# Fancomi2017/InstanceFusion

Hardware: AMD Instinct MI355X
Metric: frames/s + ms/frame (ICP|fuse|instance) at 640x480, 5M surfels, 1/2/4/8 GPU (higher is better)
Workload: dtype f32; 1 GPU; 5000000-surfel map, 640x480 synthetic RGBD stream, 3-level ICP+RGB + surfel fuse + canned-mask instance votes with superpixel refinement; surfels_live=4734799, surfel_slots=4734799, map_order=random, parallelism=replicas x1, loop_frames=90

## Files before the change

### instancefusion_amd/csrc/ifx_api.hip

```cpp
#include <climits>
#include "ifx_ctx.h"
#include <string.h>
#include <stdio.h>
#include <algorithm>

int ifx_tracker_external_pose(ifx* h, const float* d_pose16, float weight_mult);
int ifx_tracker_set_weight(ifx* h, float weight_mult);
int ifx_compact_enqueue(ifx* h, int refresh_ids);

void hs_invalidate_view(ifx* h);
static std::string g_err;
extern "C" const char* ifx_global_error(void) { return g_err.c_str(); }
extern "C" const char* ifx_last_error(ifx_t* h) { return h ? h->err.c_str() : g_err.c_str(); }

hipEvent_t ifx_event_get(ifx* h)
{
    if (!h->event_pool.empty()) { hipEvent_t e = h->event_pool.back(); h->event_pool.pop_back(); return e; }
    hipEvent_t e;
    hipEventCreate(&e);
    return e;
}
void ifx_ktime_begin(ifx* h, const char* name, hipEvent_t* a)
{
    (void)name;
// ... 285 lines not shown
    else if (s == "stage_timing") h->opt_stage_timing = value;
    else if (s == "track_ahead") h->opt_track_ahead = value;
    else if (s == "slic_ahead") h->opt_slic_ahead = value;
    else if (s == "fold_result") h->opt_fold_result = value;
    else if (s == "clean_raster") h->opt_clean_raster = value;
    else if (s == "hot_records") { h->opt_hot = value; h->hot_valid = 0; }
    else if (s == "hot_verify") h->opt_hot_verify = value;
    else if (s == "own_first_live") h->opt_own_first_live = value;
    else if (s == "own_track_rows") {
        if (!h->own) { h->err = "own_track_rows: the handle was not created for a sharded map"; return IFX_E_STATE; }
        h->opt_own_track_rows = value;
    }
    else if (s == "own_track_rows_emulate") h->opt_own_track_rows_emulate = value;
    else if (s == "own_key_rs") {
        if (!h->own) { h->err = "own_key_rs: the handle was not created for a sharded map"; return IFX_E_STATE; }
        if (h->own_g * 8 > IFX_KEY_SLACK) { h->err = "own_key_rs: more ranks than the key image's slack allows"; return IFX_E_INVALID; }
        h->opt_own_key_rs = value;
    }
    else if (s == "own_lazy_ids") {
        if (!h->own) { h->err = "own_lazy_ids: the handle was not created for a sharded map"; return IFX_E_STATE; }
        if (value && ifx_own_lattice(h) + 1 > 16 * 1024) { h->err = "own_lazy_ids: the image's id lattice is larger than the pack kernel's one workgroup holds (16 383 entries)"; return IFX_E_INVALID; }
        h->opt_own_lazy_ids = value;
    }
    else if (s == "id_rule") {
        if (value != 0 && value != 1) { h->err = "id_rule must be 0 (ray-disc) or 1 (the reference's screen-space quads)"; return IFX_E_INVALID; }
        if (h->own || h->shard_n > 1) { h->err = "id_rule: the id renders of a sharded map keep the ray-disc rule"; return IFX_E_STATE; }
        if (h->hint_rgb || h->slot[h->tick & 1].for_tick == h->tick || h->ids_pending || h->clean_raster_pending) { h->err = "id_rule cannot change while a frame is in flight or announced ahead"; return IFX_E_STATE; }
        if (value != h->opt_id_rule) {
            h->opt_id_rule = value;
            h->ids_full_valid = 0; h->ids_sparse_frame = 1; h->ids_view_ok = 0;
            h->seg_counts_valid = 0;
            const int r = ifx_ids_ensure(h);
            if (r) return r;
        }
    }
    else if (s == "cam_swap") h->opt_cam_swap = value;
    else if (s == "cam_side") h->opt_cam_side = value;
    else if (s == "host_entry_async") h->opt_host_entry_async = value;
    else if (s == "gn_prologue_blocks") h->opt_gn_prologue_blocks = value;
    else if (s == "compact_divisor") h->opt_compact_divisor = value;
    else if (s == "icp_blocks") h->opt_icp_blocks = std::max(0, std::min(2048, value));
    else if (s == "view_blocks") h->opt_view_blocks = std::max(0, std::min(65536, value));
    else if (s == "clean_blocks") h->opt_clean_blocks = std::max(0, std::min(65536, value));
    else if (s == "index_blocks") h->opt_index_blocks = std::max(0, std::min(8192, value));
    else if (s == "res_blocks") h->opt_res_blocks = std::max(0, std::min(4096, value));
    else if (s == "rgb_blocks") h->opt_rgb_blocks = std::max(0, std::min(1024, value));
    else if (s == "raster_tiles") h->opt_raster_tiles = value;
    else if (s == "view_list") { h->opt_vlist = value; ifx_vlist_reap(h); hs_invalidate_view(h); }
    else if (s == "seg_aside") h->opt_seg_aside = value;
    else if (s == "pace") h->opt_pace = value;
    else if (s == "lazy_ids") { ifx_ids_ensure(h); h->opt_lazy_ids = value; }
    else if (s == "seg_device") h->opt_seg_device = value;
    else if (s == "compare_map") {
        if (value != 1 && value != 2) { h->err = "compare_map must be 1 (box IoU) or 2 (mask IoU)"; return IFX_E_INVALID; }
        if (value == 2 && (h->own || h->shard_n > 1)) { h->err = "compare_map 2: the mask rule is not offered on a sharded map (dilated presence is not additive over ranks)"; return IFX_E_STATE; }
        h->opt_compare_map = value;
    }
    else if (s == "seg_snapshots") { if (value < 1 || value > 8) { h->err = "seg_snapshots must be in [1, 8]"; return IFX_E_INVALID; } h->opt_seg_snapshots = value; }
    else if (s == "ff_rounds") h->opt_ff_rounds = value;
    else if (s == "gn_persist_blocks") { if (value < 1) return IFX_E_INVALID; ifx_drop_tracked(h); h->opt_gn_persist_blocks = value; }
    else if (s == "gn_persist") {
        if (value < 0 || value > 7) { h->err = "gn_persist is a mask of pyramid levels (0..7)"; return IFX_E_INVALID; }
        ifx_drop_tracked(h);
        h->opt_gn_persist = value;
    }
    else if (s == "gn_spin_limit" || s == "gn_fault") {
        if (value < 0) return IFX_E_INVALID;
        ifx_drop_tracked(h);
        HIPCHK(h, hipStreamSynchronize(h->stream));
        HIPCHK(h, hipMemcpy((char*)h->d_state + (s == "gn_fault" ? offsetof(DevState, gn_fault) : offsetof(DevState, gn_spin_limit)), &value, sizeof(int), hipMemcpyHostToDevice));
    }
    else if (s == "gn_prologue") { ifx_drop_tracked(h); h->opt_gn_prologue = value ? 1 : 0; }
    else if (s == "rgb_cand") { ifx_drop_tracked(h); h->opt_rgb_cand = value ? 1 : 0; }
    else if (s == "rgb_fuse") {
        if (value < 0 || value > 7) { h->err = "rgb_fuse is a mask of pyramid levels (0..7)"; return IFX_E_INVALID; }
        ifx_drop_tracked(h);
        h->opt_rgb_fuse = value;
    }
    else if (s == "rgb_fuse_poll") { ifx_drop_tracked(h); h->opt_rgb_fuse_poll = value ? 1 : 0; }
    else if (s == "rgb_own") {
        if (value < 0 || value > 7) { h->err = "rgb_own is a mask of pyramid levels (0..7)"; return IFX_E_INVALID; }
        ifx_drop_tracked(h);
        h->opt_rgb_own = value;
    }
    else if (s == "raster_lds") h->opt_raster_lds = value;
    else if (s == "raster_earlyz") h->opt_raster_earlyz = value;
    else if (s == "pyramid" || s == "fast_odom" || s == "so3" || s == "icp_weight_x1000") {
        if (h->hint_rgb || h->slot[h->tick & 1].for_tick == h->tick) { h->err = "tracker options cannot change while a frame is announced ahead"; return IFX_E_STATE; }
        ifx_drop_tracked(h);
        if (s == "pyramid") h->cfg.pyramid = value ? 1 : 0;
        else if (s == "fast_odom") h->cfg.fast_odom = value ? 1 : 0;
        else if (s == "so3") h->cfg.so3 = value ? 1 : 0;
        else { if (value < 0 || value > 100000) { h->err = "icp_weight_x1000 must be in [0, 100000]"; return IFX_E_INVALID; } h->cfg.icp_weight = value / 1000.f; }
    }
    else { h->err = "unknown option " + s; return IFX_E_INVALID; }
    return IFX_OK;
}

__global__ void k_frame_result(DevState* __restrict__ st, FrameResult* __restrict__ out, float* __restrict__ traj_slot)
{
    if (threadIdx.x < 64) frame_result_wave(st, out, traj_slot, 0, (int)threadIdx.x);
}

static int enqueue_frame_side(ifx* h, int s, int tick, const uint8_t* rgb, const uint16_t* depth, int src_kind)
{
    FrameSlot& f = h->slot[s];
    const int bound = h->cur_slot;
    hipStream_t q = h->opt_two_streams ? h->stream_b : h->stream;
    if (q != h->stream) HIPCHK(h, hipStreamWaitEvent(q, f.released, 0));
    if (f.snap_pending) { if (q != h->stream) HIPCHK(h, hipStreamWaitEvent(q, f.snap_read, 0)); f.snap_pending = 0; }
    h->cur = q;
    ifx_bind_slot(h, s);
    hipMemcpyKind kind = src_kind ? hipMemcpyHostToDevice : hipMemcpyDeviceToDevice;
    hipError_t e2 = hipMemcpyAsync(f.depth_raw, depth, (size_t)h->P * 2, kind, q), e1 = hipSuccess;
    if (e2 == hipSuccess) {
        StageTimer t(h, 3);
        ifx_preprocess(h);
        if (h->late_rgb_src && src_kind == 1) { memcpy(h->rgb_stage, h->late_rgb_src, (size_t)h->P * 3); h->late_rgb_src = nullptr; }
        e1 = hipMemcpyAsync(f.rgb, rgb, (size_t)h->P * 3, kind, q);
        if (e1 == hipSuccess) ifx_tracker_frame_side(h, tick == 1);
    }
    hipEventRecord(f.ready, q);
    f.for_tick = tick; f.src_rgb = rgb; f.src_depth = depth;
    h->cur = h->stream;
    ifx_bind_slot(h, bound);
    if (e1 != hipSuccess || e2 != hipSuccess) { h->err = "frame copy failed"; return IFX_E_HIP; }
    return IFX_OK;
}

int ifx_enqueue_hinted_frame_side(ifx* h)
{
    if (!h->hint_rgb || !h->opt_two_streams) { h->hint_rgb = nullptr; return IFX_OK; }
    const uint8_t* r = h->hint_rgb; const uint16_t* d = h->hint_depth;
    const int kind = h->hint_kind;
    h->hint_rgb = nullptr; h->hint_depth = nullptr; h->hint_kind = 0;
    if (h->stream_b && h->slot[h->tick & 1].ready) HIPCHK(h, hipStreamWaitEvent(h->stream_b, h->slot[h->tick & 1].ready, 0));
    int rr = enqueue_frame_side(h, (h->tick + 1) & 1, h->tick + 1, r, d, kind);
    if (!rr && kind == 1) h->prestaged_tick = h->tick + 1;
    return rr;
}

__global__ void k_lc_idle(DevState* st, float* __restrict__ host_lc)
{
    if (threadIdx.x != 0) return;
    for (int k = 0; k < 23; k++) st->lc[k] = 0.f;
    for (int k = 0; k < 16; k++) st->lc[6 + k] = st->pose[k];
    st->lc[23] = (float)st->lc_candidates;
    for (int k = 0; k < 24; k++) host_lc[k] = st->lc[k];
}
static int enqueue_loop_closure_renders(ifx* h)
{
    h->lc_deferred = 0;
    if (!h->fern_cb && !h->map_external && h->tick - h->cfg.time_delta < 1) {
        LAUNCH(h, "lc_idle", dim3(1), dim3(64), k_lc_idle, h->d_state, h->h_lc);
        return IFX_OK;
    }
    if (h->lc_pending) { HIPCHK(h, hipStreamWaitEvent(h->stream, h->ev_lc_done, 0)); h->lc_pending = 0; }
    {
        StageTimer t(h, 1);
        ifx_tracker_m2m_begin(h);
        ifx_map_predict_loop_closure(h);
    }
    if (h->fern_cb) {
        HIPCHK(h, hipStreamSynchronize(h->stream));
        h->in_fern_cb = 1;
        int r = h->fern_cb(h, h->fern_user);
// ... 1143 lines not shown
```

### instancefusion_amd/csrc/ifx_ctx.h

```cpp
#pragma once
#include <hip/hip_runtime.h>
#include <stdint.h>
#include <string>
#include <vector>
#include <map>
#include "../../include/ifx_c_api.h"
#include "ifx_dev.h"

#ifndef IFX_LIST_SEGS
#define IFX_LIST_SEGS 8
#endif

struct DevState {
    float pose[16];
    float pose_inv[16];
    float last_pose[16];
    float weighting;
    int dense_enough;
    int count;
    int n_dead;
    int n_new;
    int overflow;
    unsigned int r_max_bits;
    float Rprev[9], tprev[3], Rprev_inv[9];
// ... 228 lines not shown
    int opt_own_lazy_ids = 0;
    int opt_own_key_rs = 0;
    int opt_own_track_rows = 0, opt_own_track_rows_emulate = 0;
    int track_rc = 0;
    int own_ids_lat = 0;
    int own_ids_pending = 0;
    unsigned long long* own_lat_tmp = nullptr;
    int own_need_decide = 0;
    int pred_root = -1;
    int own_track_rank = -1;
    float own_frame_pose[16]; int own_frame_pose_set = 0;
    int own = 0, own_g = 1;
    size_t pred_bytes = 0; int* pred_tail = nullptr;
    void* comm = nullptr;
    int shard_rank = 0, shard_n = 1;
    int opt_two_streams = 1;
    int opt_stage_timing = 0;
    int opt_gn_prologue_blocks = 2048;
    int opt_cam_side = 1;
    int opt_cam_swap = 1;
    void* hot = nullptr;
    int hot_valid = 0;
    int opt_hot_verify = 0;
    int opt_hot = 1;
    void* frame_hot = nullptr;
    int opt_clean_raster = 1;
    int clean_raster_pending = 0;
    float frame_weight_mult = 1.f;
    int opt_fold_result = 1;
    float* result_fold_traj = nullptr;
    int result_folded = 0;
    int opt_slic_ahead = 1;
    int opt_track_ahead = 1;
    int tracked_ahead = 0;
    int opt_own_first_live = 1;
    int opt_pace = 1;
    int opt_seg_aside = 1;
    hipEvent_t ev_result = nullptr;
    int n_side_prepared = 0, n_tracked_ahead = 0, n_host_hinted = 0;
    int hint_kind = 0;
    uint8_t* hint_stage_rgb[2] = {nullptr, nullptr}; uint16_t* hint_stage_depth[2] = {nullptr, nullptr};
    const void *hinted_src_rgb[2] = {nullptr, nullptr}, *hinted_src_depth[2] = {nullptr, nullptr};
    int hinted_tick[2] = {-1, -1};
    const uint8_t* hint_rgb = nullptr;
    const uint16_t* hint_depth = nullptr;
    std::string err;
    int tick = 1;
    int ids_pending = 0;
    int ids_view_ok = 0;
    int view_scan_tick = -1;
    int opt_id_rule = 0;
    int opt_lazy_ids = 1;
    int ids_full_valid = 1, ids_sparse_frame = 0;
    int ids_full_hint = 0;
    int opt_compact_every_frame = 0;
    int last_compact_tick = -1;
    int opt_compact_divisor = 8;
    int opt_kernel_timing = 0;
    int opt_reference_passes = 0;
    int opt_gn_persist_blocks = 128;
    int opt_gn_persist = 0;
    int gn_max_blocks[4] = {0, 0, 0, 0};
    int opt_rgb_blocks = 0;
    int opt_gn_prologue = 1;
    int oseg_state = 0, oseg_nm = 0, oseg_m = 0, oseg_flags = 0, oseg_pending = 0;
    std::vector<uint8_t> oseg_unavail;
    std::vector<int> oseg_cmp, oseg_bbox, oseg_class;
    hipEvent_t oseg_ev = nullptr;
    int32_t* oseg_rec = nullptr;
    size_t oseg_rec_cap = 0, oseg_rec_bytes = 0;
    int oseg_root = -1, oseg_form = 0, oseg_M = 0, oseg_maxn = 0;
    float oseg_thr = 0.f;
    const char* oseg_who = "";
    void* d_kexp = nullptr;
    int gn_begin_folded = 0;
    int labels_stale_all = 1;
    int opt_raster_lds = 0;
    int opt_view_blocks = 0, opt_clean_blocks = 0, opt_index_blocks = 0;
    int icp_resident_blocks = 1024;
    int opt_res_blocks = 0;
    int opt_rgb_cand = 1;
    int opt_rgb_fuse = 7;
    int opt_rgb_own = 7;
    int opt_rgb_fuse_poll = 1;
    int icp_resident_blocks_fuse = 1024;
    int opt_icp_blocks = 0;
    int opt_raster_tiles = -1;
    int map_external = 0;
    int lc_enable = 0, lc_count_thresh = 35000;
    float lc_err_thresh = 5e-5f, lc_cov_thresh = 1e-5f;
    DevState* d_m2m = nullptr;
    Pyr m2m;
    float *old_vertex = nullptr, *old_normal = nullptr;
    uint8_t *old_image = nullptr, *old_inst = nullptr;
    uint16_t* old_time = nullptr;
    float *act_vertex = nullptr, *act_normal = nullptr;
    uint8_t *act_image = nullptr, *act_inst = nullptr;
    uint16_t* act_time = nullptr;
    size_t lc_half = 0;
    int own_tracked_tick = 0;
    float* h_lc = nullptr;
    int lc_event_valid = 0;
    float* d_graph = nullptr;
    int graph_nodes = 0, graph_is_fern = 0;
    uint8_t* d_inst_gt = nullptr;
    int inst_gt_on = 0;
    void* d_fern = nullptr;
    float* d_project = nullptr;
    float *d_sample = nullptr, *d_cons = nullptr;
    ifx_loop_closure_cb lc_cb = nullptr;
    void* lc_user = nullptr;
    ifx_fern_cb fern_cb = nullptr;
    void* fern_user = nullptr;
    uint8_t* h_fern = nullptr;
    hipEvent_t ev_fern = nullptr;
    int fern_pending = 0;
    int in_fern_cb = 0;
    DevState* d_state = nullptr;
    FrameResult* h_result = nullptr;
    float* h_pose_early = nullptr;
    hipEvent_t ev_pose_early = nullptr;
    int want_early_pose = 0, early_pose_valid = 0, housekeeping_due = 0;
    int prestaged_tick = -1;
    int opt_host_entry_async = 0;
    float* d_traj = nullptr;
    int max_traj = 1 << 16;
    float* d_scratch = nullptr;
    int n_traj = 0;
    float *pc = nullptr, *nr = nullptr, *col = nullptr, *tm = nullptr, *ic = nullptr, *votes = nullptr;
    float *pc2 = nullptr, *nr2 = nullptr, *col2 = nullptr, *tm2 = nullptr, *ic2 = nullptr, *votes2 = nullptr;
    uint32_t* upd_owner = nullptr;
    uint8_t* assoc_vis = nullptr;
    uint32_t *list_v = nullptr, *list_vi = nullptr;
    int view_frame = 0;
    int view_block = 0;
    int age_epoch = 0;
    int last_clean_time = 0;
    int view_dirty = 0;
    int opt_vlist = 1;
    int opt_raster_earlyz = 0;
    uint32_t *list_a = nullptr, *list_b = nullptr, *list_c = nullptr;
    unsigned int *tile_n = nullptr, *tile_box = nullptr, *tile_pairs = nullptr;
    unsigned int tile_pair_cap = 0;
    void* tile_recs = nullptr;
    unsigned int* d_list_ctr = nullptr;
    unsigned int list_seg_cap = 0;
    int32_t *labels = nullptr, *labels2 = nullptr;
    uint32_t *seq = nullptr, *seq2 = nullptr;
    int* scan_flags = nullptr;
    int* scan_block = nullptr;
    int* scan_out = nullptr;
    uint8_t* rgb = nullptr;
    uint16_t *depth_raw = nullptr, *depth_filt = nullptr;
    float *dm = nullptr, *dmf = nullptr;
    uint8_t* rgb_stage = nullptr; uint16_t* depth_stage = nullptr;
    const uint8_t* late_rgb_src = nullptr;
    unsigned long long *key_index = nullptr, *key_splat = nullptr, *key_ids = nullptr;
    unsigned long long* key_both = nullptr;
    uint32_t* index_id = nullptr;
    float *index_vc = nullptr, *index_ct = nullptr, *index_nr = nullptr, *index_tap = nullptr;
    float *pred_vertex = nullptr, *pred_normal = nullptr, *pred_conf = nullptr;
    uint8_t *pred_image = nullptr, *pred_inst = nullptr;
    uint16_t* pred_time = nullptr;
    float *fill_vertex = nullptr, *fill_normal = nullptr;
    uint8_t* fill_image = nullptr;
    int32_t *ids_after = nullptr, *ids_tmp = nullptr;
// ... 148 lines not shown
```

### instancefusion_amd/csrc/ifx_track.hip

```cpp
#include "ifx_ctx.h"
#include "ifx_rgb_chunks.h"
#include "ifx_rgb_own.h"
#include <math.h>
#include <string.h>


#define BIL_R 6
#define BIL_BX 32
#define BIL_BY 8
template <bool SHIFTED, bool XCLIP>
__device__ __forceinline__ void bil_window(const uint16_t (*tile)[BIL_BX + 2 * BIL_R + 3], const unsigned char* s_mapx, const unsigned char* s_mapy, int x, int y, int bx, int by, int tx1,
                                           int ty1, unsigned int value, float& sum1, float& sum2)
{
    const float ss = 0.024691358f, sc = 0.000555556f;
    constexpr int D = BIL_R * 2 + 1;
    const float fv = (float)value;
    for (int cy = max(y - D / 2, 0); cy < ty1; ++cy) {
        const int ry = SHIFTED ? (int)s_mapy[cy - by + BIL_R + 1] : cy - by + BIL_R + 1;
        const float dy = (float)y - (float)cy, dy2 = dy * dy;
        float tv[D];
#pragma unroll
        for (int q = 0; q < D; q++) {
            const int col = x - D / 2 + q - bx + BIL_R + 1;
            tv[q] = (float)tile[ry][SHIFTED ? (int)s_mapx[col] : col];
        }
#pragma unroll
        for (int q = 0; q < D; q += 2) {
            const int cx = x - D / 2 + q;
            const bool ok0 = !XCLIP || (cx >= 0 && cx < tx1), ok1 = q + 1 < D && (!XCLIP || (cx + 1 >= 0 && cx + 1 < tx1));
            ifx_v2f dxv, t2;
            dxv.x = (float)x - (float)cx; dxv.y = (float)x - (float)(cx + 1);
            t2.x = tv[q]; t2.y = q + 1 < D ? tv[q + 1] : 0.f;
            const ifx_v2f space2 = dxv * dxv + dy2;
            const ifx_v2f dv = fv - t2;
            const ifx_v2f color2 = dv * dv;
            const ifx_v2f wgt = ifx_expf2_nonpos(-(space2 * ss + color2 * sc));
            if (ok0) { sum1 += t2.x * wgt.x; sum2 += wgt.x; }
            if (ok1) { sum1 += t2.y * wgt.y; sum2 += wgt.y; }
        }
    }
}
__global__ __launch_bounds__(BIL_BX* BIL_BY) void k_bilateral_metric(const uint16_t* __restrict__ in, uint16_t* __restrict__ filt,
                                                                      float* __restrict__ dm, float* __restrict__ dmf, int w, int h, float maxD)
{
    __shared__ uint16_t tile[BIL_BY + 2 * BIL_R + 1][BIL_BX + 2 * BIL_R + 3];
    __shared__ unsigned char s_mapx[BIL_BX + 2 * BIL_R + 1], s_mapy[BIL_BY + 2 * BIL_R + 1];
    __shared__ int s_shifted;
    const int bx = blockIdx.x * BIL_BX, by = blockIdx.y * BIL_BY;
    const int tid = threadIdx.y * BIL_BX + threadIdx.x;
    const int TW = BIL_BX + 2 * BIL_R + 1, TH = BIL_BY + 2 * BIL_R + 1;
    if (tid == 0) s_shifted = 0;
    __syncthreads();
    for (int i = tid; i < TW * TH; i += BIL_BX * BIL_BY) {
        int ty = i / TW, tx = i - ty * TW;
        int gx = bx + tx - BIL_R - 1, gy = by + ty - BIL_R - 1;
        uint16_t v = 0;
        if (gx >= 0 && gx < w && gy >= 0 && gy < h) v = in[gy * w + gx];
        tile[ty][tx] = v;
    }
    if (tid < TW) {
        const int gx = bx + tid - BIL_R - 1;
        int t = tid;
        if (gx >= 0 && gx < w) t = max(min(max((int)floorf(((float)gx / (float)w) * (float)w), 0), w - 1) - (bx - BIL_R - 1), 0);
        s_mapx[tid] = (unsigned char)t;
        if (t != tid) s_shifted = 1;
    }
    if (tid >= 64 && tid - 64 < TH) {
        const int k = tid - 64, gy = by + k - BIL_R - 1;
        int t = k;
        if (gy >= 0 && gy < h) t = max(min(max((int)floorf(((float)gy / (float)h) * (float)h), 0), h - 1) - (by - BIL_R - 1), 0);
        s_mapy[k] = (unsigned char)t;
        if (t != k) s_shifted = 1;
    }
    __syncthreads();
    const int x = bx + threadIdx.x, y = by + threadIdx.y;
    if (x >= w || y >= h) return;
    const unsigned int maxv = (unsigned int)(maxD * 1000.0f);
    unsigned int value = tile[threadIdx.y + BIL_R + 1][threadIdx.x + BIL_R + 1];
    unsigned int outv = 0;
    if (!(value > maxv || value < 300u)) {
        const float ss = 0.024691358f, sc = 0.000555556f;
        const int D = BIL_R * 2 + 1;
        int tx1 = min(x - D / 2 + D, w), ty1 = min(y - D / 2 + D, h);
        float sum1 = 0, sum2 = 0;
        const bool shifted = s_shifted != 0, xclip = bx < BIL_R || bx + BIL_BX + BIL_R > w;
// ... 1876 lines not shown
#endif
    __syncthreads();
#ifdef IFX_STAMPS
    long long ts_c = clock64();
#endif
    if (threadIdx.x >= 64 && threadIdx.x < 128) {
        gn_diagnostics(st, threadIdx.x - 64, s_res, s_oi, s_or, s_sys, icp, rgb, true, final_iter != 0);
        return;
    }
    if (threadIdx.x != 0) return;
    float Rc[9], tc[3], krk[9], kt[3];
    gn_serial_lane(s_sys, icp, RRt, Rp, tp, nfx, nfy, ncx, ncy, ki, Rc, tc, krk, kt);
    gn_publish_pose(st, RRt, Rc, tc, krk, kt);
    if (end_run) track_end_vals(st, rgb, 1, Rc, tc, Rp, tp, weight_mult, commit, lctr);
#ifdef IFX_STAMPS
    { long long ts_d = clock64(); st->dbg[4] += ts_d - ts_c; st->dbg[6] += ts_b - ts_a; st->dbg[7] += ts_c - ts_b; st->dbg[3] += ts_a; }
#endif
}


struct StepArgs {
    const Corres8* corres;
    const float* cloud;
    float fx, fy, sobelScale;
    const int16_t *dIdx, *dIdy;
    int w, h, nb, nb_icp, nb_res;
    int icp, rgb;
    float icp_weight, nfx, nfy, ncx, ncy;
    KInv ki;
    int check_skip;
    int final_iter;
    int end_run, commit;
    float weight_mult;
    unsigned int* lctr;
    int pro, pro_k;
};
template <bool CHECK_SKIP, bool LIST = false>
__global__ __launch_bounds__(RED_THREADS) void k_rgb_step_solve(DevState* st, int nb, int rgb, int w, int h, StepArgs a, const CandEntry* __restrict__ cand, const unsigned int* __restrict__ cand_n)
{
    __builtin_assume(st != nullptr);
    if (CHECK_SKIP && st->skip) return;
    const int par = a.pro_k & 1, set = a.pro_k % 3;
    int* const res_total = a.pro ? st->gnp_res + set * 16 : st->gn_res;
    unsigned int* const ticket = &st->gn_ticket;
    double* const icp_acc = a.pro ? st->gnp_acc + (size_t)(set * 2) * IFX_ACC_REPL * IFX_ACC_STRIDE : st->gn_acc;
    double* const rgb_acc = icp_acc + IFX_ACC_REPL * IFX_ACC_STRIDE;
    __shared__ int s_last;
    if (a.pro && blockIdx.x == 0) {
        for (int d = 1; d <= (a.pro == 2 ? 2 : 1); d++) {
            const int cs = (a.pro_k + d) % 3;
            gnp_clear_set(st->gnp_acc + (size_t)(cs * 2) * IFX_ACC_REPL * IFX_ACC_STRIDE, st->gnp_res + cs * 16, st->gnp_meet + cs * 32, &st->range_exceeded);
        }
    }
#ifdef IFX_STAMPS
    long long t0 = clock64();
#endif
    if (rgb) {
        if (LIST) rgb_step_cand_body(blockIdx.x, nb, a.corres, cand, cand_n, a.cloud, a.fx, a.fy, a.sobelScale, w, h, rgb_acc, res_total);
        else rgb_step_body(blockIdx.x, nb, a.corres, 0.f, nullptr, 0, a.cloud, a.fx, a.fy, a.dIdx, a.dIdy, a.sobelScale, w, h, rgb_acc, res_total);
    }
    if (a.pro == 1) return;
    asm volatile("s_waitcnt vmcnt(0)" ::: "memory");
    __syncthreads();
#ifdef IFX_STAMPS
    long long t1 = clock64();
#endif
    if (threadIdx.x == 0) {
        unsigned int t = __hip_atomic_fetch_add(ticket, 1u, __ATOMIC_RELAXED, __HIP_MEMORY_SCOPE_AGENT);
        s_last = (t == (unsigned int)(nb - 1));
    }
    __syncthreads();
    if (!s_last) return;
    if (threadIdx.x == 0) __hip_atomic_store(ticket, 0u, __ATOMIC_RELAXED, __HIP_MEMORY_SCOPE_AGENT);
#ifdef IFX_STAMPS
    long long t2 = clock64();
#endif
    gn_solve_block(st, icp_acc, rgb_acc, nullptr, 0, a.icp, rgb, a.icp_weight, a.nfx, a.nfy, a.ncx, a.ncy, a.ki, res_total, a.final_iter, a.end_run, a.weight_mult, a.commit, a.lctr,
                   (a.pro && a.pro_k > 0) ? st->gnp_RRt[1 - par] : (const double*)nullptr);
#ifdef IFX_STAMPS
    if (threadIdx.x == 0) { long long t3 = clock64(); st->dbg[0] += t2 - t0; st->dbg[1] += t3 - t2; st->dbg[2] += 1; st->dbg[5] += t1 - t0; st->dbg[3] -= t2; g_dbg2[0] += s_dbg_blk[0]; g_dbg2[1] += s_dbg_blk[1]; g_dbg2[2] += s_dbg_blk[2]; }
#endif
}


__global__ __launch_bounds__(RED_THREADS, 4) void k_icp_residual_rows(const DevState* __restrict__ st, int nb_icp, int w, int h, double* __restrict__ gacc, int* __restrict__ gres, PairArgs a,
                                                                      int srank, int sn)
{
    __builtin_assume(st != nullptr);
    if ((int)blockIdx.x < nb_icp) {
        IcpArgs ia;
        icp_body<false, true, false>(blockIdx.x * sn + srank, nb_icp * sn, st, ia, a.vmap_curr, a.nmap_curr, a.vmap_prev, a.nmap_prev, a.fx, a.fy, a.cx, a.cy, a.distThres, a.angleThres, w, h, gacc);
    } else {
        ResArgs ra;
        residual_body<true, false>(blockIdx.x - nb_icp, a.nb_res, st, ra, a.minScale, a.dIdx, a.dIdy, a.lastDepth, a.nextDepth, a.lastImage, a.nextImage, a.corres, a.maxDepthDelta, w, h, nullptr, gres);
    }
}
__global__ __launch_bounds__(RED_THREADS) void k_rgb_step_rows(DevState* st, int nb, int w, int h, StepArgs a, int srank, int sn)
{
    __builtin_assume(st != nullptr);
    rgb_step_body(blockIdx.x * sn + srank, nb * sn, a.corres, 0.f, nullptr, 0, a.cloud, a.fx, a.fy, a.dIdx, a.dIdy, a.sobelScale, w, h, st->gn_acc + IFX_ACC_REPL * IFX_ACC_STRIDE, st->gn_res);
}
__global__ __launch_bounds__(RED_THREADS) void k_gn_solve_rows(DevState* st, StepArgs a)
{
    __builtin_assume(st != nullptr);
    gn_solve_block(st, st->gn_acc, st->gn_acc + IFX_ACC_REPL * IFX_ACC_STRIDE, nullptr, 0, a.icp, a.rgb, a.icp_weight, a.nfx, a.nfy, a.ncx, a.ncy, a.ki, st->gn_res, a.final_iter, a.end_run, a.weight_mult,
                   a.commit, a.lctr, (const double*)nullptr);
}

struct LevelArgs {
    const float *vmap_curr, *nmap_curr, *vmap_prev, *nmap_prev;
    const int16_t *dIdx, *dIdy;
    const float *lastDepth, *nextDepth;
    const uint8_t *lastImage, *nextImage;
    const float* cloud;
    Corres8* corres;
    float fx, fy, cx, cy, distThres, angleThres, minScale, maxDepthDelta, sobelScale;
    int w, h, iters, icp, rgb;
    float icp_weight;
    float nfx, nfy, ncx, ncy;
    KInv ki_same, ki_next;
    int acc_base;
    int level;
    int final_level;
    int commit;
    float weight_mult;
    unsigned int* lctr;
};

struct GnLevelLds {
    double RRt[16];
    double sys[27];
    float pose[24];
    float oi[29], orr[29];
    int res[2];
};
__device__ __forceinline__ void gn_level_lds_begin(GnLevelLds& s, const DevState* st)
{
    const int tid = threadIdx.x;
    if (tid < 9) { s.pose[tid] = st->Rcurr[tid]; s.pose[12 + tid] = st->krkinv[tid]; }
    if (tid < 3) { s.pose[9 + tid] = st->tcurr[tid]; s.pose[21 + tid] = st->kt[tid]; }
    if (tid < 16) s.RRt[tid] = st->resultRt[tid];
}
template <bool SINGLE>
__device__ __forceinline__ void gn_level_tail(DevState* st, const LevelArgs& a, GnLevelLds& s, int bid, bool last_it, double* icp_acc, double* rgb_acc, int rcnt, int rsig,
                                              const float (&Rp)[9], const float (&tpv)[3])
{
    const int tid = threadIdx.x;
    if (tid < 29) {
        const double ti = acc_total(icp_acc, tid), tr = acc_total(rgb_acc, tid);
        if (SINGLE) { acc_clear(icp_acc, tid); acc_clear(rgb_acc, tid); }
        if (bid == 0) range_note(st, range_exceeded7(0, tid, ti), range_exceeded7(1, tid, tr));
        const float oi = (float)ti, orr = (float)tr;
        s.oi[tid] = oi; s.orr[tid] = orr;
        if (tid < 27) s.sys[tid] = gn_system_entry(tid, oi, orr, 1, 1, a.icp_weight);
    }
    if (tid == 64) { s.res[0] = rcnt; s.res[1] = rsig; }
    __syncthreads();
    if (bid == 0 && last_it && a.final_level && tid >= 64 && tid < 128) gn_diagnostics(st, tid - 64, s.res, s.oi, s.orr, s.sys, 1, 1, true, true);
    if (tid == 0 && !(last_it && bid != 0)) {
        double RRt[16];
#pragma unroll
        for (int k = 0; k < 16; k++) RRt[k] = s.RRt[k];
        float Rc[9], tcn[3], krkn[9], ktn[3];
        if (last_it) gn_serial_lane(s.sys, 1, RRt, Rp, tpv, a.nfx, a.nfy, a.ncx, a.ncy, a.ki_next, Rc, tcn, krkn, ktn);
        else gn_serial_lane(s.sys, 1, RRt, Rp, tpv, a.fx, a.fy, a.cx, a.cy, a.ki_same, Rc, tcn, krkn, ktn);
#pragma unroll
// ... 599 lines not shown
    return la;
}

static void emit_rows_run(TrackRun& r)
{
    ifx* const h = r.h;
    DevState* const st = r.st;
    const Pyr& p = r.p;
    const int icp = r.plan.icp, rgb = r.plan.rgb;
    double* const gacc = gn_acc_of(st);
    int* const gres = gn_res_of(st);
    const int Ge = h->opt_own_track_rows_emulate > 1 ? h->opt_own_track_rows_emulate : 0;
    const int sn = Ge ? Ge : h->own_g, r_lo = Ge ? 0 : h->cfg.rank, r_hi = Ge ? Ge : h->cfg.rank + 1;
    const int row = IFX_ACC_REPL * IFX_ACC_STRIDE;
    for (int i = IFX_NUM_PYRS - 1; i >= 0; i--) {
        if (i == 0) ifx_enqueue_hinted_frame_side(h);
        const int lw = p.w[i], lh = p.h[i], n = lw * lh;
        const int nbv = cdiv(red_blocks(h, n), sn), nbr = std::min(cdiv(n, RED_THREADS * RED_IT), h->res_rows);
        const int nb_rgb_v = cdiv(std::min(red_blocks(h, n, RED_IT_RGB), h->opt_rgb_blocks > 0 ? h->opt_rgb_blocks : 192), sn);
        PairArgs pa = pair_args(r, i);
        pa.nb_icp = icp ? nbv : 0; pa.nb_res = rgb ? nbr : 0; pa.check_skip = 0;
        for (int j = 0; j < r.plan.iterations[i]; j++) {
            for (int q = r_lo; q < r_hi; q++) {
                const int grid = pa.nb_icp + (q == r_lo ? pa.nb_res : 0);
                if (grid > 0)
                    LAUNCH(h, icp_name_rows(i), dim3(grid), dim3(RED_THREADS), k_icp_residual_rows, (const DevState*)st, pa.nb_icp, lw, lh, gacc, gres, pa, q, sn);
            }
            if (icp && h->track_rc == IFX_OK) h->track_rc = ifx_comm_allreduce_f64(h, gacc, row);
            StepArgs sa2 = step_args(r, i, j);
            sa2.nb = nb_rgb_v; sa2.nb_icp = pa.nb_icp; sa2.nb_res = pa.nb_res; sa2.check_skip = 0; sa2.lctr = h->d_list_ctr; sa2.pro = 0; sa2.pro_k = 0;
            r.ended = r.ended || sa2.end_run;
            if (rgb) {
                for (int q = r_lo; q < r_hi; q++) LAUNCH(h, "rgb_step_rows", dim3(nb_rgb_v), dim3(RED_THREADS), k_rgb_step_rows, st, nb_rgb_v, lw, lh, sa2, q, sn);
                if (h->track_rc == IFX_OK) h->track_rc = ifx_comm_allreduce_f64(h, gacc + row, row);
            }
            LAUNCH(h, "gn_solve_rows", dim3(1), dim3(RED_THREADS), k_gn_solve_rows, st, sa2);
        }
    }
}

struct LevelLaunch {
    PairArgs pa;
    int nb, nb_rgb, nbr;
    const CandEntry* cl;
    const unsigned int* cln;
};
static LevelLaunch level_launch(const TrackRun& r, int i)
{
    ifx* const h = r.h;
    const Pyr& p = r.p;
    const bool cand_run = r.plan.cand_run;
    LevelLaunch L;
    const int n = p.w[i] * p.h[i];
    L.nb = red_blocks(h, n);
    L.nb_rgb = cand_run ? rgb_cand_blocks(h, n, i, true) : std::min(red_blocks(h, n, RED_IT_RGB), h->opt_rgb_blocks > 0 ? h->opt_rgb_blocks : 192);
    const int res_round = std::max(128, h->icp_resident_blocks - (r.plan.icp ? L.nb : 0));
    L.nbr = cand_run ? rgb_cand_blocks(h, n, i, false) : std::min(std::min(cdiv(n, RED_THREADS * RED_IT), h->res_rows), h->opt_res_blocks > 0 ? h->opt_res_blocks : res_round);
    L.cl = cand_run ? p.cand[i] : nullptr;
    L.cln = cand_run ? p.cand_n[i] : nullptr;
    L.pa = pair_args(r, i);
    L.pa.nb_icp = r.plan.icp ? L.nb : 0; L.pa.nb_res = r.plan.rgb ? L.nbr : 0; L.pa.check_skip = r.frame_tracker ? 0 : 1;
    return L;
}
static void emit_persistent_level(TrackRun& r, int i, const PairArgs& pa)
{
    ifx* const h = r.h;
    static const decltype(&k_gn_level<1>) kernel[4] = {k_gn_level<1>, k_gn_level<2>, k_gn_level<3>, k_gn_level<4>};
    const LevelArgs la = level_args(pa, r, i);
    r.persist_iters += r.plan.iterations[i];
    LAUNCH(h, "gn_level", dim3(r.plan.persist_nb[i]), dim3(RED_THREADS), kernel[r.plan.persist_q[i]], r.st, la);
    LAUNCH(h, "gn_level_solo", dim3(1), dim3(RED_THREADS), k_gn_level_solo, r.st, la);
    r.ended = r.ended || la.final_level;
}
static void emit_iteration(TrackRun& r, int i, int j, const LevelLaunch& L)
{
    ifx* const h = r.h;
    DevState* const st = r.st;
    const RunPlan& pl = r.plan;
    const PairArgs& pa = L.pa;
    const int tail_k = r.tail_k++;
    GnPro gp;
    gp.k = tail_k; gp.icp = pl.icp; gp.rgb = pl.rgb; gp.icp_weight = r.icp_weight; gp.nfx = pa.fx; gp.nfy = pa.fy; gp.ncx = pa.cx; gp.ncy = pa.cy; gp.ki = kinv_of(pa.fx, pa.fy, pa.cx, pa.cy);
    const bool it_pro = pl.pro && tail_k < pl.n_pro;
    const bool fuse = pl.cand_run && it_pro && tail_k < pl.n_pro - 1 && (h->opt_rgb_fuse & (1 << i));
    double* const ga = it_pro ? gnp_acc_of(st, tail_k % 3) : gn_acc_of(st);
    int* const gr = it_pro ? gnp_res_of(st, tail_k % 3) : gn_res_of(st);
    double* const rrt_store = gnp_rrt_of(st, (tail_k + 1) & 1);
    FuseArgs fa;
    memset(&fa, 0, sizeof(fa));
    PairArgs paf = pa;
    if (fuse) {
        paf.nb_res = std::max(1, std::min(rgb_fuse_blocks(h, pa.w * pa.h), h->icp_resident_blocks_fuse - pa.nb_icp));
        const int cs = (tail_k + 1) % 3;
        fa.cloud = r.p.cloud[i]; fa.sobelScale = (float)GN_SOBEL_SCALE; fa.g = paf.nb_res; fa.poll_ticks = h->opt_rgb_fuse_poll ? RGB_MEET_TICKS : 0u;
        fa.meet = gnp_meet_of(st, tail_k % 3); fa.clear_acc = gnp_acc_of(st, cs); fa.clear_res = gnp_res_of(st, cs); fa.clear_meet = gnp_meet_of(st, cs);
        fa.range_ctr = (int*)((char*)st + offsetof(DevState, range_exceeded)); fa.giveups = (int*)((char*)st + offsetof(DevState, rgb_meet_giveups));
        fa.adopted = (int*)((char*)st + offsetof(DevState, rgb_meet_adopted));
    }
    const bool own = fuse && (h->opt_rgb_own & (1 << i)) && paf.nb_res <= RGB_OWN_MAX_G;
    LAUNCH(h, icp_name(i), dim3(paf.nb_icp + paf.nb_res), dim3(RED_THREADS), icp_residual_kernel(!r.frame_tracker, it_pro && tail_k > 0, pl.cand_run, fuse, own), st, paf.nb_icp, paf.w, paf.h, ga, gr, paf,
           gp, rrt_store, L.cl, L.cln, fa);
    if (fuse) return;
    StepArgs sa2 = step_args(r, i, j);
    sa2.nb = L.nb_rgb; sa2.nb_icp = L.nb; sa2.nb_res = L.nbr; sa2.check_skip = r.frame_tracker ? 0 : 1; sa2.lctr = r.frame_tracker ? h->d_list_ctr : (unsigned int*)nullptr;
    sa2.pro = it_pro ? (tail_k == pl.n_pro - 1 ? 2 : 1) : 0; sa2.pro_k = tail_k;
    r.ended = r.ended || sa2.end_run;
    LAUNCH(h, rgb_name(i), dim3(L.nb_rgb), dim3(RED_THREADS), rgb_step_solve_kernel(!r.frame_tracker, pl.cand_run), st, sa2.nb, sa2.rgb, sa2.w, sa2.h, sa2, L.cl, L.cln);
}

static void tracker_run(ifx* h, DevState* st, Pyr& p, float icp_weight, int so3, float weight_mult, int commit, bool frame_tracker, int keep_last = 0)
{
    const ifx_config& c = h->cfg;
    TrackRun r = {h, st, p, icp_weight, weight_mult, commit, frame_tracker, plan_run(h, p, icp_weight, frame_tracker), 0, 0, false};
    const RunPlan& pl = r.plan;
    if (frame_tracker && h->gn_begin_folded) h->gn_begin_folded = 0;
    else {
        const float div = (float)(1 << (pl.first < 0 ? 0 : pl.first));
        LAUNCH(h, "track_gn_begin", dim3(1), dim3(64), k_track_gn_begin, st, h->slot[h->cur_slot].so3, so3, c.fx / div, c.fy / div, c.cx / div, c.cy / div, keep_last, h->opt_gn_persist ? 1 : 0);
    }
    if (frame_tracker && h->own && h->opt_own_track_rows && ifx_comm_ready(h) && h->own_track_rank < 0) emit_rows_run(r);
    else
        for (int i = IFX_NUM_PYRS - 1; i >= 0; i--) {
            if (i == 0 && frame_tracker) ifx_enqueue_hinted_frame_side(h);
            const LevelLaunch L = level_launch(r, i);
            if (pl.persist_q[i] >= 0) emit_persistent_level(r, i, L.pa);
            else
                for (int j = 0; j < pl.iterations[i]; j++) emit_iteration(r, i, j, L);
        }
    if (!r.ended)
        LAUNCH(h, "track_end", dim3(1), dim3(64), k_track_end, st, pl.rgb, 1, weight_mult, commit, frame_tracker ? h->d_list_ctr : (unsigned int*)nullptr);
}

int ifx_tracker_frame_side(ifx* h, int first, double* so3_acc, unsigned int* so3_ticket)
{
    Pyr& p = h->pyr;
    const ifx_config& c = h->cfg;
    if (first) {
        LAUNCH(h, "intensity", dim3(cdiv(h->P, 256)), dim3(256), k_intensity, h->rgb, 3, h->P, p.next_img[0]);
        for (int i = 0; i + 1 < IFX_NUM_PYRS; i++)
            LAUNCH(h, "pyrdown_u8", G2(p.w[i + 1], p.h[i + 1]), B2, k_pyrdown_gauss_u8, p.next_img[i], p.w[i], p.h[i], p.next_img[i + 1]);
        return IFX_OK;
    }
    tracker_init_frame(h, h->depth_filt, h->rgb);
    if (c.so3) {
        const float d2 = 4.f;
        const int L = 2, n = p.w[L] * p.h[L], nb = cdiv(n, RED_THREADS);
        DevState* ss = h->slot[h->cur_slot].so3;
        LAUNCH(h, "so3_begin", dim3(1), dim3(64), k_so3_begin, ss, c.fx / d2, c.fy / d2, c.cx / d2, c.cy / d2);
        for (int it = 0; it < 10; it++)
            LAUNCH(h, "so3_fused", dim3(nb), dim3(RED_THREADS), k_so3_fused, ss, p.lastnext_img[L], p.next_img[L], p.w[L], p.h[L], so3_acc ? so3_acc : p.acc + 2 * IFX_ACC_REPL * IFX_ACC_STRIDE, nb,
                   so3_ticket ? so3_ticket : h->d_ticket + 4, c.fx / d2, c.fy / d2, c.cx / d2, c.cy / d2);
    }
    return IFX_OK;
}

int ifx_tracker_model_side(ifx* h, int fold_begin)
{
    const ifx_config& c = h->cfg;
    const bool fold = fold_begin && c.pyramid && IFX_NUM_PYRS == 3;
    GnBegin gb = gb_none();
    if (fold) {
        const float div = (float)(1 << (IFX_NUM_PYRS - 1));
        gb.st = h->d_state; gb.ss = h->slot[h->cur_slot].so3; gb.so3 = c.so3; gb.fx = c.fx / div; gb.fy = c.fy / div; gb.cx = c.cx / div; gb.cy = c.cy / div;
        gb.keep_last = 0; gb.enabled = 1; gb.persist = h->opt_gn_persist ? 1 : 0;
    }
    tracker_init_model(h, h->d_state, h->pyr, h->cfg.icp_weight, h->pred_vertex, h->pred_normal, h->pred_image, h->fill_vertex, h->fill_normal, h->fill_image, fold ? &gb : nullptr);
    h->gn_begin_folded = fold ? 1 : 0;
    return IFX_OK;
}

static int cam_trk_alloc(ifx* h)
{
    if (h->d_cam_trk) return IFX_OK;
    Pyr& p = h->cam_pyr;
    HIPCHK(h, hipMalloc(&h->d_cam_trk, sizeof(DevState)));
    HIPCHK(h, hipMemset(h->d_cam_trk, 0, sizeof(DevState)));
    for (int i = 0; i < IFX_NUM_PYRS; i++) {
        p.w[i] = h->w >> i; p.h[i] = h->h >> i;
        const size_t n = (size_t)p.w[i] * p.h[i];
        HIPCHK(h, hipMalloc(&p.vmap_cam[i], n * 12)); HIPCHK(h, hipMalloc(&p.nmap_cam[i], n * 12));
        HIPCHK(h, hipMalloc(&p.vmap_prev[i], n * 12)); HIPCHK(h, hipMalloc(&p.nmap_prev[i], n * 12));
        HIPCHK(h, hipMalloc(&p.last_depth[i], n * 4));
        HIPCHK(h, hipMalloc(&p.last_img[i], n));
        HIPCHK(h, hipMalloc(&p.cloud[i], n * 12));
        HIPCHK(h, hipMalloc(&p.corres[i], n * 8));
    }
    HIPCHK(h, hipMalloc(&h->cam_so3_acc, IFX_ACC_REPL * IFX_ACC_STRIDE * sizeof(double)));
    HIPCHK(h, hipMemset(h->cam_so3_acc, 0, IFX_ACC_REPL * IFX_ACC_STRIDE * sizeof(double)));
    HIPCHK(h, hipMalloc(&h->cam_so3_ticket, 64));
// ... 488 lines not shown
```

Before: 1904 frames/s.

## Fuse final chained GN iteration's RGB residual into ICP kernel with single-block finish solve

The last iteration of the prologue Gauss-Newton chain previously did not use the fused ICP+RGB residual kernel. It fell back to a separate multi-block RGB step-and-solve kernel. It now also runs the fused kernel and then launches a single-block k_gn_finish kernel, which clears the next accumulator set, resets the meet counters and solves from the fused accumulators. This replaces a full-grid RGB reduction launch with a one-block solve, at the cost of tighter coupling between the accumulator-set rotation indices and the fused kernel's clearing scheme.

```diff
diff --git a/instancefusion_amd/csrc/ifx_api.hip b/instancefusion_amd/csrc/ifx_api.hip
--- a/instancefusion_amd/csrc/ifx_api.hip
+++ b/instancefusion_amd/csrc/ifx_api.hip
@@ -391,6 +391,11 @@
         if (value < 0 || value > 7) { h->err = "rgb_own is a mask of pyramid levels (0..7)"; return IFX_E_INVALID; }
         ifx_drop_tracked(h);
         h->opt_rgb_own = value;
+    }
+    else if (s == "gn_finish") {
+        if (value < 0 || value > 1) { h->err = "gn_finish is 0 or 1"; return IFX_E_INVALID; }
+        ifx_drop_tracked(h);
+        h->opt_gn_finish = value;
     }
     else if (s == "raster_lds") h->opt_raster_lds = value;
     else if (s == "raster_earlyz") h->opt_raster_earlyz = value;
diff --git a/instancefusion_amd/csrc/ifx_ctx.h b/instancefusion_amd/csrc/ifx_ctx.h
--- a/instancefusion_amd/csrc/ifx_ctx.h
+++ b/instancefusion_amd/csrc/ifx_ctx.h
@@ -334,6 +334,7 @@
     int opt_rgb_cand = 1;
     int opt_rgb_fuse = 7;
     int opt_rgb_own = 7;
+    int opt_gn_finish = 1;
     int opt_rgb_fuse_poll = 1;
     int icp_resident_blocks_fuse = 1024;
     int opt_icp_blocks = 0;
diff --git a/instancefusion_amd/csrc/ifx_gn_sets.h b/instancefusion_amd/csrc/ifx_gn_sets.h
--- /dev/null
+++ b/instancefusion_amd/csrc/ifx_gn_sets.h
@@ -0,0 +1,10 @@
+#pragma once
+
+#include "ifx_rgb_chunks.h"
+
+#define GN_SETS 3
+
+IFX_HD inline int gn_set_sum(int k) { return k % GN_SETS; }
+IFX_HD inline int gn_set_read(int k) { return (k - 1) % GN_SETS; }
+IFX_HD inline int gn_set_clear(int k) { return (k + 1) % GN_SETS; }
+IFX_HD inline int gn_set_clear_last(int k) { return (k + 2) % GN_SETS; }
diff --git a/instancefusion_amd/csrc/ifx_track.hip b/instancefusion_amd/csrc/ifx_track.hip
--- a/instancefusion_amd/csrc/ifx_track.hip
+++ b/instancefusion_amd/csrc/ifx_track.hip
@@ -1,6 +1,7 @@
 #include "ifx_ctx.h"
 #include "ifx_rgb_chunks.h"
 #include "ifx_rgb_own.h"
+#include "ifx_gn_sets.h"
 #include <math.h>
 #include <string.h>
 
@@ -2043,6 +2044,22 @@
 #endif
 }
 
+template <bool CHECK_SKIP>
+__global__ __launch_bounds__(RED_THREADS) void k_gn_finish(DevState* st, StepArgs a)
+{
+    __builtin_assume(st != nullptr);
+    if (CHECK_SKIP && st->skip) return;
+    const int par = a.pro_k & 1, set = gn_set_sum(a.pro_k), cs = gn_set_clear_last(a.pro_k);
+    double* const icp_acc = st->gnp_acc + (size_t)(set * 2) * IFX_ACC_REPL * IFX_ACC_STRIDE;
+    unsigned int* const meet = st->gnp_meet + set * 32;
+    gnp_clear_set(st->gnp_acc + (size_t)(cs * 2) * IFX_ACC_REPL * IFX_ACC_STRIDE, st->gnp_res + cs * 16, st->gnp_meet + cs * 32, &st->range_exceeded);
+    if (threadIdx.x >= 192 && threadIdx.x < 194) __hip_atomic_store(&meet[(threadIdx.x - 192) * 16], 0u, __ATOMIC_RELAXED, __HIP_MEMORY_SCOPE_AGENT);
+    if (threadIdx.x >= 194 && threadIdx.x < 196)
+        __hip_atomic_store(reinterpret_cast<unsigned long long*>(meet + RGB_MEET_ORPHAN) + (threadIdx.x - 194), 0ull, __ATOMIC_RELAXED, __HIP_MEMORY_SCOPE_AGENT);
+    gn_solve_block(st, icp_acc, icp_acc + IFX_ACC_REPL * IFX_ACC_STRIDE, nullptr, 0, a.icp, a.rgb, a.icp_weight, a.nfx, a.nfy, a.ncx, a.ncy, a.ki, st->gnp_res + set * 16, a.final_iter, a.end_run,
+                   a.weight_mult, a.commit, a.lctr, st->gnp_RRt[1 - par]);
+}
+
 
 __global__ __launch_bounds__(RED_THREADS, 4) void k_icp_residual_rows(const DevState* __restrict__ st, int nb_icp, int w, int h, double* __restrict__ gacc, int* __restrict__ gres, PairArgs a,
                                                                       int srank, int sn)
@@ -2808,7 +2825,8 @@
     GnPro gp;
     gp.k = tail_k; gp.icp = pl.icp; gp.rgb = pl.rgb; gp.icp_weight = r.icp_weight; gp.nfx = pa.fx; gp.nfy = pa.fy; gp.ncx = pa.cx; gp.ncy = pa.cy; gp.ki = kinv_of(pa.fx, pa.fy, pa.cx, pa.cy);
     const bool it_pro = pl.pro && tail_k < pl.n_pro;
-    const bool fuse = pl.cand_run && it_pro && tail_k < pl.n_pro - 1 && (h->opt_rgb_fuse & (1 << i));
+    const bool chain_end = it_pro && tail_k == pl.n_pro - 1;
+    const bool fuse = pl.cand_run && it_pro && (!chain_end || h->opt_gn_finish) && (h->opt_rgb_fuse & (1 << i));
     double* const ga = it_pro ? gnp_acc_of(st, tail_k % 3) : gn_acc_of(st);
     int* const gr = it_pro ? gnp_res_of(st, tail_k % 3) : gn_res_of(st);
     double* const rrt_store = gnp_rrt_of(st, (tail_k + 1) & 1);
@@ -2826,11 +2844,16 @@
     const bool own = fuse && (h->opt_rgb_own & (1 << i)) && paf.nb_res <= RGB_OWN_MAX_G;
     LAUNCH(h, icp_name(i), dim3(paf.nb_icp + paf.nb_res), dim3(RED_THREADS), icp_residual_kernel(!r.frame_tracker, it_pro && tail_k > 0, pl.cand_run, fuse, own), st, paf.nb_icp, paf.w, paf.h, ga, gr, paf,
            gp, rrt_store, L.cl, L.cln, fa);
-    if (fuse) return;
+    if (fuse && !chain_end) return;
     StepArgs sa2 = step_args(r, i, j);
     sa2.nb = L.nb_rgb; sa2.nb_icp = L.nb; sa2.nb_res = L.nbr; sa2.check_skip = r.frame_tracker ? 0 : 1; sa2.lctr = r.frame_tracker ? h->d_list_ctr : (unsigned int*)nullptr;
-    sa2.pro = it_pro ? (tail_k == pl.n_pro - 1 ? 2 : 1) : 0; sa2.pro_k = tail_k;
+    sa2.pro = it_pro ? (chain_end ? (fuse ? 3 : 2) : 1) : 0; sa2.pro_k = tail_k;
     r.ended = r.ended || sa2.end_run;
+    if (fuse) {
+        if (r.frame_tracker) LAUNCH(h, rgb_name(i), dim3(1), dim3(RED_THREADS), k_gn_finish<false>, st, sa2);
+        else LAUNCH(h, rgb_name(i), dim3(1), dim3(RED_THREADS), k_gn_finish<true>, st, sa2);
+        return;
+    }
     LAUNCH(h, rgb_name(i), dim3(L.nb_rgb), dim3(RED_THREADS), rgb_step_solve_kernel(!r.frame_tracker, pl.cand_run), st, sa2.nb, sa2.rgb, sa2.w, sa2.h, sa2, L.cl, L.cln);
 }
 
```

Result: no change. 1913 frames/s (median of 2 runs) (+0.5%).
